# RajeshRk18/exacto

Hardware: AMD Instinct MI355X
Metric: ciphertext muls/sec (bfv_mul_and_relin) (higher is better)
Workload: dtype u64; 1 GPU; bfv_mul_and_relin, BASELINE configs[2]; ring_degree=4096, ct_limbs=3, limb_bits=60, plain_modulus=65537, gadget_base=65536, gadget_digits=12, batch_per_gpu=1024, global_batch=1024, parallelism=batch-shard x1

## Files before the change

### exacto_amd/csrc/arith.hpp

```cpp
#pragma once
#include <hip/hip_runtime.h>
#include <stdint.h>

typedef uint64_t u64;
typedef int64_t i64;
typedef unsigned __int128 u128;
typedef __int128 i128;

#define EXACTO_MAX_L 8
#define EXACTO_MAX_K 10
#define EXACTO_MAX_PRIMES (EXACTO_MAX_L + EXACTO_MAX_K)
#define EXACTO_MAX_G 64

struct __attribute__((aligned(16))) TwPair {
    u64 w;
    u64 ws;
};

struct PrimeConst {
    u64 q, two_q;
    u64 mu64;
    u64 bar_mu;
    int bar_s;
    int pad_;
    u64 n_inv, n_inv_s;
    u64 last_w, last_ws;
    const TwPair* tw_fwd;
    const TwPair* tw_inv;
    u64 qinv_neg;
    u64 n_inv_r, n_inv_rs, last_wr, last_wrs;
};

__device__ __forceinline__ u64 mont_mul_lazy(u64 a, u64 b, u64 q, u64 qinv_neg) {
    const u64 lo = a * b, hi = __umul64hi(a, b);
    const u64 m = lo * qinv_neg;
    return hi + __umul64hi(m, q) + (lo != 0 ? 1 : 0);
}

__device__ __forceinline__ u64 mulhi64(u64 y, u64 s) {
    const uint32_t y0 = (uint32_t)y, y1 = (uint32_t)(y >> 32);
    const uint32_t s0 = (uint32_t)s, s1 = (uint32_t)(s >> 32);
    const u64 u = (u64)y1 * s0 + __umulhi(y0, s0);
    const u128 v = (u128)((u64)y0 * s1) + u;
    return (u64)y1 * s1 + (u64)(v >> 32);
}

// ... 75 lines not shown
```

### exacto_amd/csrc/context.hip

```cpp
#include <algorithm>
#include <cxxabi.h>
#include <dlfcn.h>
#include <chrono>
#include <condition_variable>
#include <cmath>
#include <cstdio>
#include <cstdlib>
#include <cstring>
#include <functional>
#include <map>
#include <memory>
#include <mutex>
#include <set>
#include <string>
#include <thread>
#include <vector>

#include "../../include/exacto_hip.h"
#include "exacto_internal.hpp"

using namespace exacto;

thread_local const void* exacto::g_last_kernel = nullptr;

// ... 648 lines not shown

static int build_tables(exacto_ctx* c) {
    const int NP = (int)c->primes.size();
    std::vector<TwPair> tw((size_t)NP * 2 * c->n);
    std::vector<PrimeConst> pc(NP);
    for (int t = 0; t < NP; ++t)
        pc[t] = make_prime_const(c->primes[t], c->n, c->logn, &tw[(size_t)t * 2 * c->n],
                                 &tw[(size_t)t * 2 * c->n + c->n]);
    HIP_TRY(dev_alloc((void**)&c->d_tw, tw.size() * sizeof(TwPair)));
    if (int e_ = upload(c, c->d_tw, tw.data(), tw.size() * sizeof(TwPair))) return e_;
    for (int t = 0; t < NP; ++t) {
        pc[t].tw_fwd = c->d_tw + (size_t)t * 2 * c->n;
        pc[t].tw_inv = c->d_tw + (size_t)t * 2 * c->n + c->n;
    }
    HIP_TRY(dev_alloc((void**)&c->d_primes, NP * sizeof(PrimeConst)));
    if (int e_ = upload(c, c->d_primes, pc.data(), NP * sizeof(PrimeConst))) return e_;

    CrtTables& C = c->h_crt;
    std::memset(&C, 0, sizeof(C));
    const int L = c->L, K = c->K;
    C.L = L;
    C.K = K;
    C.G = c->G;
    C.gbase = c->gbase;
    C.gshift = (c->gbase & (c->gbase - 1)) == 0 ? bitlen(c->gbase) - 1 : -1;
    C.plain = c->plain;
    const std::vector<u64> qv(c->primes.begin(), c->primes.begin() + L);
    const std::vector<u64> pv(c->primes.begin() + L, c->primes.end());
    for (int i = 0; i < L; ++i)
        for (int k = 0; k < i; ++k) set_shoup(C.gq_w[i][k], C.gq_ws[i][k], invmod_h(qv[k] % qv[i], qv[i]), qv[i]);
    Big Q(1);
// ... 80 lines not shown
                for (int b = 0; b < K; ++b)
                    if (b != a) pm = mulmod_h(pm, pv[b] % qv[i], qv[i]);
                C.fpc_pm[a][i] = pm;
            }
        }
        for (int i = 0; i < L; ++i) {
            const u64 pm = P.mod(qv[i]);
            C.fpc_negP[i] = pm == 0 ? 0 : qv[i] - pm;
        }
        for (int i = 0; i < L; ++i) {
            const u64 q = qv[i];
            u64 qo = 1 % q;
            for (int k = 0; k < L; ++k)
                if (k != i) qo = mulmod_h(qo, qv[k] % q, q);
            set_shoup(C.fpq_pz_w[i], C.fpq_pz_ws[i], mulmod_h(c->plain % q, invmod_h(qo, q), q), q);
            C.fpq_inv0[i] = 1.0 / (double)q;
            C.fpq_inv1[i] = (double)(1ull << 30) / (double)q;
            for (int a = 0; a < K; ++a) {
                const u64 pa = pv[a], qi = invmod_h(q % pa, pa);
                C.fpq_c[i][a] = mulmod_h((pa - qi) % pa, C.fpc_neg[a], pa);
            }
        }
    }
    {
        const u64 mx = *std::max_element(c->primes.begin(), c->primes.end());
        const u64 mn = *std::min_element(c->primes.begin(), c->primes.end());
        C.near = (u128)mx < 2 * (u128)mn;
        C.fast = C.near && mx < (1ull << 60);
        C.special = C.fast && mn > (1ull << 60) - (1ull << 24);
        C.digit_small = c->gbase <= *std::min_element(qv.begin(), qv.end());
    }
    HIP_TRY(dev_alloc((void**)&c->d_scal, EXACTO_MAX_L * sizeof(u64)));
    HIP_TRY(dev_alloc((void**)&c->d_crt, sizeof(CrtTables)));
    if (int e_ = upload(c, c->d_crt, &C, sizeof(CrtTables))) return e_;
    return 0;
}

extern "C" int exacto_ctx_create(exacto_ctx** out, size_t n, const uint64_t* ct_moduli, size_t L,
// ... 341 lines not shown
            CHECK_LAUNCH();
            return 0;
        }
    }
    if (int e = run_ntt(c, nb1, count1, false)) return e;
    return run_ntt(c, nb2, count2, false);
}

static bool tensor_asm(const exacto_ctx* c) {
    bool near60 = c->ntt_asm && c->ntt_asm_inv;
    for (int t = 0; t < c->L + c->K; ++t)
        near60 &= c->primes[t] < (1ull << 60) && c->primes[t] > (1ull << 60) - (1ull << 24);
    return near60;
}

static int run_inv_tensor(exacto_ctx* c, const Operands& o, int cnt, bool p2only = false) {
    const int NP = c->L + c->K;
    bool lazy = true;
    const bool near60 = tensor_asm(c);
    int qbits = 0;
    for (int t = 0; t < NP; ++t) {
        qbits = std::max(qbits, 64 - __builtin_clzll(c->primes[t]));
        lazy &= c->primes[t] < (1ull << 60);
    }
    const double pb = 8.0 * c->n;
    double bytes;
    if (c->tensor_share_d > 0 && c->tensor_share_npairs > 0) {
        const double items = (double)((cnt + c->tensor_share_npairs - 1) / c->tensor_share_npairs);
        const double cts = items * 2.0 * c->tensor_share_d;
        bytes = pb * (c->L * (2.0 * cts + 3.0 * cnt) +
                      c->K * (p2only ? cts + (double)cnt : 2.0 * cts + 3.0 * cnt));
    } else {
        bytes = cnt * (p2only ? pb * (7.0 * c->L + 3.0 * c->K) : pb * 7.0 * NP);
    }
    ProfScope ps(c, PK_TENSOR, (u64)cnt * (p2only ? 3 * c->L + c->K : 3 * NP), bytes);
    launch_inv_tensor(o, c->ws_extP, c->ws_T, cnt, c->logn, c->L, c->K, lazy, c->d_primes, c->stream, near60, p2only,
                      qbits, c->tensor_share_npairs, near60 && c->path != EXACTO_PATH_HPS);
    CHECK_LAUNCH();
    return 0;
}

static NttBatch contiguous(u64* data, long count_items, long poly_per_item, int prime_base, int period,
                           int n) {
    (void)count_items;
    NttBatch nb{};
    nb.src = data;
    nb.src_off = nullptr;
    nb.src_item_stride = poly_per_item * n;
    nb.dst = data;
    nb.dst_item_stride = poly_per_item * n;
    nb.ppi = (int)poly_per_item;
    nb.prime_base = prime_base;
// ... 235 lines not shown
                ProfScope pl(c, PK_HPS_EXT, 4ull * cnt, 8.0 * (1 + K) * n * 4.0 * cnt);
                launch_hps_extend(c->ws_coefQ, c->ws_extP, 4L * cnt, n, c->d_primes, K, c->stream);
            } else {
                ProfScope pl(c, PK_LIFT, 4ull * cnt, 8.0 * (L + K) * n * 4.0 * cnt);
                launch_exact_lift(c->ws_coefQ, c->ws_extP, 4L * cnt, n, c->d_crt, c->d_primes, L, K,
                                  crt_mode(c), c->stream);
            }
            CHECK_LAUNCH();
            NttBatch eb = contiguous(c->ws_extP, cnt, 4L * K, L, K, n);
            eb.lazy_out = c->path != EXACTO_PATH_HPS && tensor_asm(c);
            if (int e = run_ntt(c, eb, (long)cnt * 4 * K, false)) return e;
        } else {
            o.ea_off += s;
            o.eb_off += s;
        }
        if (int e = run_inv_tensor(c, o, cnt, ps.on)) return e;
        if (ps.on) {
            const int ib_cnt = cnt / ps.npairs;
            {
                ProfScope pp(c, PK_PAIRSUM, (u64)ib_cnt * K * ps.d, 8.0 * n * K * ib_cnt * (4.0 * ps.d + 2.0 * ps.d));
                launch_dbfv_pairsum(o, c->ws_extP, ib_cnt, ps.d, ps.npairs, ps.term_start, ps.terms, L, K, n,
                                    c->d_primes, c->stream);
            }
            CHECK_LAUNCH();
            if (int e = run_ntt(c, contiguous(c->ws_extP, (long)ib_cnt * ps.d, 2L * K, L, K, n),
                                (long)ib_cnt * ps.d * 2 * K, true))
                return e;
        }
        u64* R = out + s * out_stride;
        const int ncomp = relin ? 2 : 3;
        u64* D = relin ? c->ws_D : nullptr;
// ... 5 lines not shown
        if (c->path == EXACTO_PATH_HPS) {
            void* d16p = hps_defer ? (c->ks_defer8 ? (void*)((int8_t*)c->ks_defer + s * (long)guse * n)
                                                   : (void*)(c->ks_defer + s * (long)guse * n))
                                   : nullptr;
            launch_hps_scale(c->ws_T, R, out_stride, ncomp, hps_defer ? nullptr : D, d16p,
                             hps_defer && c->ks_defer8, guse, cnt, n, c->d_crt, c->d_primes, K, c->hps_fast,
                             c->stream);
        } else
            launch_exact_scale(c->ws_T, R, out_stride, ncomp, d16 ? nullptr : D,
                               d16 ? (c->ks_defer ? (c->ks_defer8
                                                         ? (int16_t*)((int8_t*)c->ks_defer + s * (long)guse * n)
                                                         : c->ks_defer + s * (long)guse * n)
                                                  : c->ws_D16)
                                   : nullptr,
                               guse, cnt, n, c->d_crt, c->d_primes, L, K, crt_mode(c),
                               c->stream, c->h_crt.gshift, ps.on, c->ks_defer && c->ks_defer8, c->fp_crt, c->fpq_lim);
        CHECK_LAUNCH();
        }
        if (ps.on) {
            const long item0 = s / ps.npairs;
            const double ib = (double)(cnt / ps.npairs);
            ProfScope pq(c, PK_PSUM_SCALE, (u64)(cnt / ps.npairs) * ps.d,
                         ib * 2.0 * n * 8.0 * (ps.d * (double)(K + L) + (double)ps.npairs * L));
            if (!launch_psum_scale(c->ws_T, c->ws_extP, ps.out + item0 * ps.d * 2 * Ln, cnt / ps.npairs, ps.d, ps.npairs,
                                   ps.term_start, ps.terms, n, c->d_crt, c->d_primes, L, c->stream, ps.fpc,
                                   c->fpq_lim))
                return fail(EXACTO_ERR_HIP, "internal: psum scale not available for these limbs");
            CHECK_LAUNCH();
        }
        NttBatch rb{};
        rb.src = R; rb.src_off = nullptr; rb.src_item_stride = out_stride;
// ... 2963 lines not shown
```

### exacto_amd/csrc/exacto_internal.hpp

```cpp
#pragma once
#include "arith.hpp"

namespace exacto {

struct NttBatch {
    const u64* src;
    const u64* src_off;
    long src_item_stride;
    u64* dst;
    long dst_item_stride;
    int ppi;
    int prime_base;
    int period;
    const int16_t* src16;
    long src16_item_stride;
    int lazy_out;
};

enum class MulPath : int { Exact = 0, Hps = 1 };

struct CrtTables {
    int L;
    int K;
    int G;
// ... 10 lines not shown
    u64 halfP_mr[EXACTO_MAX_K];
    u64 ppref_w[EXACTO_MAX_K + 1][EXACTO_MAX_L];
    u64 ppref_ws[EXACTO_MAX_K + 1][EXACTO_MAX_L];
    u64 qinvp_w[EXACTO_MAX_K], qinvp_ws[EXACTO_MAX_K];
    u64 pq_w[EXACTO_MAX_K], pq_ws[EXACTO_MAX_K];
    u64 qpq_w[EXACTO_MAX_L + 1][EXACTO_MAX_K], qpq_ws[EXACTO_MAX_L + 1][EXACTO_MAX_K];
    u64 fpc_pq[EXACTO_MAX_K];
    u64 fpc_qpq[EXACTO_MAX_L][EXACTO_MAX_K];
    u64 fpc_neg[EXACTO_MAX_K];
    double fpc_inv[EXACTO_MAX_K];
    u64 fpc_pm[EXACTO_MAX_K][EXACTO_MAX_L];
    u64 fpc_negP[EXACTO_MAX_L];
    u64 fpq_pz_w[EXACTO_MAX_L], fpq_pz_ws[EXACTO_MAX_L];
    double fpq_inv0[EXACTO_MAX_L], fpq_inv1[EXACTO_MAX_L];
    u64 fpq_c[EXACTO_MAX_L][EXACTO_MAX_K];
    int near;
    int fast;
    int special;
    int digit_small;
    u64 pmod_w[EXACTO_MAX_PRIMES], pmod_ws[EXACTO_MAX_PRIMES];
    u64 Qwords[EXACTO_MAX_L];
    u64 hq[EXACTO_MAX_PRIMES];
    u64 hps_qinv[2];
    u64 hps_p1_inv_p0, hps_p0_inv_p1;
    u64 hps_pc;
    u64 hps_qinv_s[2];
    u64 hps_t_w[2], hps_t_ws[2];
    u64 hps_pq_w[2], hps_pq_ws[2];
    u64 hps_kPq[3];
    u64 hps_P[2], hps_halfP[2];
// ... 54 lines not shown
    const u64* eb;
    const u64* eb_off;
};

bool launch_polymul(const u64* A, const u64* B, u64* out, long rows, int period, int logn, const PrimeConst* primes,
                    hipStream_t s);
void launch_mul_inv(const u64* A, const u64* B, u64* out, long rows, int period, int logn, bool lazy, bool asm_inv,
                    const PrimeConst* primes, hipStream_t s);
struct DropPrimeK {
    u64 w[EXACTO_MAX_L], ws[EXACTO_MAX_L];
};
void launch_drop_prime(const u64* in, u64* out, long rows, int l, bool round, const DropPrimeK& C, int logn, bool lazy,
                       bool asm_rounds, const PrimeConst* primes, hipStream_t s);
void launch_inv_tensor(const Operands& op, const u64* extP, u64* T, int items, int logn, int L, int K, bool lazy,
                       const PrimeConst* primes, hipStream_t s, bool asm_inv = false, bool p2only = false,
                       int qbits = 64, int share_np = 0, bool lazy_out = false);
void launch_phase(const u64* ct, int polys, long ct_stride, const u64* sk, u64* out, int items, int n, int L,
                  const PrimeConst* primes, hipStream_t s);
void launch_decrypt_round(const u64* X, u64* out, int items, int n, int L, const CrtTables* ct,
                          const PrimeConst* primes, u64 plain, hipStream_t s);
int noise_chunks(int n);
void launch_noise(const u64* X, const u64* expected, u64* plain_out, u64* part, u64* out, long items, int group,
                  int n, int L, const CrtTables* ct, const PrimeConst* primes, const u64* delta, u64 plain,
                  bool round, hipStream_t s);
void launch_dbfv_recompose(const u64* digits, u64* out, int items, int n, int d, u64 base, u64 plain, u64 t,
                           bool scalar, hipStream_t s);
void launch_exact_lift(const u64* coefQ, u64* extP, long rows, int n, const CrtTables* ct,
                       const PrimeConst* primes, int L, int K, int mode, hipStream_t s);
void launch_hps_extend(const u64* coefQ, u64* extP, long rows, int n, const PrimeConst* primes,
                       int K, hipStream_t s);
bool exact_scale_sp_ok(int L, int K, int mode);
void launch_exact_scale(const u64* T, u64* R, long r_stride, int ncomp_r, u64* D, int16_t* D16, int guse,
                        int items, int n, const CrtTables* ct, const PrimeConst* primes, int L,
                        int K, int mode, hipStream_t s, int gshift = -1, bool c2only = false,
                        bool digits8 = false, bool fpc = false, double fpq_lim = 0.0);
void launch_hps_scale(const u64* T, u64* R, long r_stride, int ncomp_r, u64* D, void* D16, bool d8, int guse,
                      int items, int n, const CrtTables* ct, const PrimeConst* primes, int K, bool fast,
                      hipStream_t s);
void launch_decompose(const u64* C2, long c2_stride, u64* D, int guse, int items, int n,
                      const CrtTables* ct, const PrimeConst* primes, int L, hipStream_t s, int16_t* D16 = nullptr);
void launch_rows(u64* dst, long dst_stride, const u64* src, long src_stride, long len, long rows, hipStream_t s);
void launch_copy_u64(u64* dst, const u64* src, long words, hipStream_t s);
void launch_xcd_probe(const u64* src, u64* dst, long words, uint32_t* xcc, int blocks, hipStream_t s);
void launch_fill_u32(uint32_t* dst, uint32_t v, long words, hipStream_t s);
void debug_watch_set(const void* lo, const void* hi, uint32_t* hit, hipStream_t s = nullptr);
void launch_relin_mac(const u64* base, long base_stride, const u64* D, const u64* rlk, const u64* rlk_s,
                      int guse, u64* out, long out_stride, int items, int n, int L, const PrimeConst* primes,
                      hipStream_t s);

enum class PwOp : int { Add = 0, Sub = 1, Neg = 2, Mul = 3, ScalarMul = 4, Copy = 5 };
// ... 74 lines not shown
```

### exacto_amd/csrc/kernels.hip

```cpp
#include "exacto_internal.hpp"
#include "crt_dev.hpp"

#include <cstdlib>

namespace exacto {

static constexpr int TPB = 256;

static inline int blocks_per_row(int n) { return (n + TPB - 1) / TPB; }

#define ROW_SETUP(n)                                                   \
    const int nblk = (n + TPB - 1) / TPB;                              \
    const int nsh = __builtin_ctz((unsigned)nblk);                     \
    const long row = (long)(blockIdx.x >> nsh);                        \
    const int j = (int)(blockIdx.x & (unsigned)(nblk - 1)) * TPB + threadIdx.x; \
    if (j >= (n)) return;




template <bool SP>
__device__ __forceinline__ u64 reduce_any(u64 x, const PrimeConst& P) {
    return SP ? reduce_near60(x, P.q) : reduce64(x, P.q, P.mu64);
}
// ... 413 lines not shown
        y0[a] = (uint32_t)y[a] & M30;
        y1[a] = (uint32_t)(y[a] >> 30);
    }
    const uint32_t alpha = (uint32_t)__double2int_rn(f);
#pragma unroll
    for (int i = 0; i < L; ++i) {
        const u64 q = primes[i].q;
        Dot30 A{0, 0, 0};
        dot30_mac(A, alpha, 0, C->fpc_negP[i]);
#pragma unroll
        for (int a = 0; a < K; ++a) dot30_mac(A, y0[a], y1[a], C->fpc_pm[a][i]);
        res[i] = dot30_fold(A, q);
    }
}

template <int LT, bool TA>
__device__ __forceinline__ void fpc_y_garner(const u64* __restrict__ Tin, int n, u64 (&y)[LT + 1],
                                             const CrtTables* __restrict__ C, const PrimeConst* __restrict__ primes) {
    constexpr int L = LT, K = LT + 1;
    u64 u[EXACTO_MAX_L], v[EXACTO_MAX_L];
#pragma unroll
    for (int i = 0; i < L; ++i) u[i] = shoup_mul(Tin[(long)i * n], C->pmod_w[i], C->pmod_ws[i], primes[i].q);
    garner_q_fast<LT>(v, u, L, C, primes);
    const bool negs = mr_greater<EXACTO_MAX_L>(v, C->halfQ_mr, L);
    uint32_t v0[L], v1[L];
#pragma unroll
    for (int k = 0; k < L; ++k) {
        v0[k] = (uint32_t)v[k] & M30;
        v1[k] = (uint32_t)(v[k] >> 30);
    }
#pragma unroll
    for (int a = 0; a < K; ++a) {
        Dot30 A{(TA ? 0ull : y[a]) + (negs ? C->fpc_neg[a] : 0ull), 0, 0};
        if constexpr (TA) {
            const u64 ta = Tin[(long)(L + a) * n];
            dot30_mac(A, (uint32_t)ta & M30, (uint32_t)(ta >> 30), C->fpc_pq[a]);
        }
#pragma unroll
        for (int k = 0; k < L; ++k) dot30_mac(A, v0[k], v1[k], C->fpc_qpq[k][a]);
        y[a] = dot30_fold(A, primes[L + a].q);
    }
}

template <int LT, bool TA>
__device__ __forceinline__ void fpq_y(const u64* __restrict__ Tin, int n, u64 (&y)[LT + 1], const CrtTables* __restrict__ C,
                                      const PrimeConst* __restrict__ primes, double lim) {
    constexpr int L = LT, K = LT + 1;
    uint32_t z0[L], z1[L];
    double f = 0.0;
#pragma unroll
    for (int i = 0; i < L; ++i) {
        const u64 z = shoup_mul_red(Tin[(long)i * n], C->fpq_pz_w[i], C->fpq_pz_ws[i], primes[i].q);
        z0[i] = (uint32_t)z & M30;
        z1[i] = (uint32_t)(z >> 30);
        f = fma((double)z0[i], C->fpq_inv0[i], f);
        f = fma((double)z1[i], C->fpq_inv1[i], f);
    }
    const double b = __builtin_rint(f);
    if (__builtin_fabs(f - b) <= lim) {
        const uint32_t beta = (uint32_t)b;
#pragma unroll
        for (int a = 0; a < K; ++a) {
            Dot30 A{TA ? 0ull : y[a], 0, 0};
            dot30_mac(A, beta, 0, C->fpc_neg[a]);
            if constexpr (TA) {
                const u64 ta = Tin[(long)(L + a) * n];
                dot30_mac(A, (uint32_t)ta & M30, (uint32_t)(ta >> 30), C->fpc_pq[a]);
            }
#pragma unroll
            for (int i = 0; i < L; ++i) dot30_mac(A, z0[i], z1[i], C->fpq_c[i][a]);
            y[a] = dot30_fold(A, primes[L + a].q);
        }
    } else {
        fpc_y_garner<LT, TA>(Tin, n, y, C, primes);
    }
}

template <int LT>
__device__ __forceinline__ void fpq_acc(const u64* __restrict__ Tin, int n, u64 (&Z)[LT], uint32_t& bs, u64 (&carry)[LT + 1],
                                        const CrtTables* __restrict__ C, const PrimeConst* __restrict__ primes,
                                        double lim) {
    constexpr int L = LT;
    u64 z[L];
    double f = 0.0;
#pragma unroll
    for (int i = 0; i < L; ++i) {
        z[i] = shoup_mul_red(Tin[(long)i * n], C->fpq_pz_w[i], C->fpq_pz_ws[i], primes[i].q);
        f = fma((double)((uint32_t)z[i] & M30), C->fpq_inv0[i], f);
        f = fma((double)(uint32_t)(z[i] >> 30), C->fpq_inv1[i], f);
// ... 29 lines not shown
        Z[i] = 0;
    }
#pragma unroll
    for (int a = 0; a < K; ++a) {
        const u64 pa = primes[L + a].q;
        Dot30 A{carry[a], 0, 0};
        dot30_mac(A, bs, 0, C->fpc_neg[a]);
        dot30_mac(A, ks, 0, pa - C->fpc_neg[a]);
#pragma unroll
        for (int i = 0; i < L; ++i) dot30_mac(A, z0[i], z1[i], C->fpq_c[i][a]);
        carry[a] = dot30_fold(A, pa);
    }
    bs = 0;
}

template <int LT, int DIG, bool FPC, bool FPQ = false>
__global__ void __launch_bounds__(TPB)
exact_scale_sp_kernel(const u64* __restrict__ T, u64* __restrict__ R, long r_stride, int ncomp_r,
                      u64* __restrict__ D, int16_t* __restrict__ D16, int guse, int n,
                      const CrtTables* __restrict__ C, const PrimeConst* __restrict__ primes, int c2only,
                      double fpq_lim = 0.0) {
    ROW_SETUP(n)
    constexpr int L = LT, K = LT + 1, NP = L + K;
    const long item = c2only ? row : row / 3;
    const int comp = c2only ? 2 : (int)(row - item * 3);
    const u64* Tin = T + (item * 3 + comp) * NP * n + j;
    u64 res[EXACTO_MAX_L];
    if constexpr (FPQ) {
        static_assert(FPC, "FPQ feeds the float lift from P");
        u64 y[K];
        fpq_y<LT, true>(Tin, n, y, C, primes, fpq_lim);
        fpc_lift<LT>(y, res, C, primes);
    } else {
    u64 u[EXACTO_MAX_L], v[EXACTO_MAX_L];
#pragma unroll
    for (int i = 0; i < L; ++i) u[i] = shoup_mul(Tin[(long)i * n], C->pmod_w[i], C->pmod_ws[i], primes[i].q);
    garner_q_fast<LT>(v, u, L, C, primes);
    const bool negs = mr_greater<EXACTO_MAX_L>(v, C->halfQ_mr, L);
    uint32_t v0[L], v1[L];
#pragma unroll
    for (int k = 0; k < L; ++k) {
        v0[k] = (uint32_t)v[k] & M30;
        v1[k] = (uint32_t)(v[k] >> 30);
    }
    if constexpr (FPC) {
        u64 y[K];
// ... 177 lines not shown
    switch (L) {
        case 1: PSUM_(1); break;
        case 2: PSUM_(2); break;
        case 3: PSUM_(3); break;
        case 4: PSUM_(4); break;
        case 5: PSUM_(5); break;
        case 6: PSUM_(6); break;
        default: return false;
    }
#undef PSUM_
    return true;
}

bool exact_scale_sp_ok(int L, int K, int mode) { return mode == 3 && K == L + 1 && L >= 1 && L <= 6 && use_dot30(); }

void launch_exact_scale(const u64* T, u64* R, long r_stride, int ncomp_r, u64* D, int16_t* D16, int guse,
                        int items, int n, const CrtTables* ct, const PrimeConst* primes, int L,
                        int K, int mode, hipStream_t s, int gshift, bool c2only, bool digits8, bool fpc,
                        double fpq_lim) {
    const long blocks = (long)items * (c2only ? 1 : 3) * blocks_per_row(n);
    if (blocks == 0) return;
    if (mode == 3 && K == L + 1 && L >= 1 && L <= 6 && use_dot30()) {
        const int dig = (D16 == nullptr && D == nullptr) || guse <= 0 ? 0
                        : (D16 != nullptr && gshift > 0 && 32 % gshift == 0) ? (digits8 && gshift <= 8 ? 3 : 1) : 2;
#define SCALE30_(LT, DG)                                                                                        \
    do {                                                                                                        \
        if (fpc && fpq_lim > 0.0)                                                                               \
            EXACTO_LAUNCH((exact_scale_sp_kernel<LT, DG, true, true>), dim3(blocks), dim3(TPB), 0, s, T, R,     \
                          r_stride, ncomp_r, D, D16, guse, n, ct, primes, c2only ? 1 : 0, fpq_lim);             \
        else if (fpc) EXACTO_LAUNCH((exact_scale_sp_kernel<LT, DG, true>), dim3(blocks), dim3(TPB), 0, s, T, R, \
                               r_stride, ncomp_r, D, D16, guse, n, ct, primes, c2only ? 1 : 0, 0.0);            \
        else EXACTO_LAUNCH((exact_scale_sp_kernel<LT, DG, false>), dim3(blocks), dim3(TPB), 0, s, T, R,         \
                           r_stride, ncomp_r, D, D16, guse, n, ct, primes, c2only ? 1 : 0, 0.0);                \
    } while (0)
#define SCALE30(LT)                         \
    do {                                    \
        if (dig == 1) SCALE30_(LT, 1);      \
        else if (dig == 3) SCALE30_(LT, 3); \
        else if (dig == 2) SCALE30_(LT, 2); \
        else SCALE30_(LT, 0);               \
    } while (0)
        switch (L) {
// ... 630 lines not shown
```

### exacto_amd/csrc/ntt.hip

```cpp
#include "exacto_internal.hpp"
#include "ks32_dev.hpp"
#include "bufmem.hpp"
#include "crt_dev.hpp"

namespace exacto {

#ifndef EXACTO_TW_AS
#define EXACTO_TW_AS 1
#endif
#if EXACTO_TW_AS == 0
typedef const TwPair* TwTab;
#else
typedef const TwPair __attribute__((address_space(EXACTO_TW_AS)))* TwTab;
#endif

__device__ __forceinline__ TwTab tw_table(const TwPair* p) { return (TwTab)p; }

__device__ __forceinline__ TwPair ld_tw(TwTab tab, int i) {
    TwPair t;
    t.w = tab[i].w;
    t.ws = tab[i].ws;
    return t;
}

// ... 191 lines not shown
#pragma unroll
    for (int k = 0; k < 16; ++k) {
        u64 v = x[k];
        if (LAZY) {
            v = v >= q8 ? v - q8 : v;
            v = v >= 4 * q ? v - 4 * q : v;
        }
        v = v >= q2 ? v - q2 : v;
        x[k] = v >= q ? v - q : v;
    }
    store_evals<N>(dst, x, tid);
}


#include "ntt_asm.inc"

template <int LO>
__device__ __forceinline__ int lds_base_bytes(int tid) {
    return swz(((tid >> LO) << (LO + 4)) | (tid & ((1 << LO) - 1))) << 3;
}

template <int LO>
__device__ __forceinline__ void lds_store_x(u64* lds, const u64 (&x)[16], int tid) {
    char* lb = reinterpret_cast<char*>(lds);
    const int b = lds_base_bytes<LO>(tid);
#pragma unroll
    for (int k = 0; k < 16; ++k) *reinterpret_cast<u64*>(lb + (b ^ (swz(k << LO) << 3))) = x[k];
}

template <int LO>
// ... 489 lines not shown
        const long ib = g / LQ;
        const int t = (int)(g - ib * LQ), c = w / np, pi = w - c * np;
        prod = ib * np + pi;
        rem = 3 * t + c;
    } else {
        const long bb = b - nQ;
        const long p = remap ? xcd_group_remap(bb, total - nQ, np) : bb;
        const long g = p / np;
        const int pi = (int)(p - g * np);
        const long ib = g / K;
        prod = ib * np + pi;
        rem = 3 * L + (int)(g - ib * K);
    }
}

template <int LOGN, bool LAZY, bool ASM = false, int PROBE = 0, bool GEN = false, int QB = 60, bool LZO = false>
__global__ void __launch_bounds__((1 << LOGN) / 16 < 64 ? 64 : (1 << LOGN) / 16)
__attribute__((amdgpu_waves_per_eu(3)))
ntt_inv_tensor_kernel(Operands op, const u64* __restrict__ extP, u64* __restrict__ Tout, int L, int K,
                      const PrimeConst* __restrict__ primes, int remap, int p2only = 0, int share_np = 0) {
    constexpr int N = 1 << LOGN;
    constexpr int T = N / 16;
    __shared__ u64 lds[N];
    const int tid = T < 64 ? vtid() : (int)threadIdx.x;
    if (tid >= T) return;
    if constexpr (PROBE == 3) probe_stagger<3>(768, EXACTO_PROBE_SLEEPS_TENSOR);
    const int NP = L + K;
    const int per = p2only ? 3 * L + K : 3 * NP;
    long item;
    int rem;
    tensor_block(blockIdx.x, gridDim.x, per, L, K, p2only, share_np, remap, item, rem);
// ... 56 lines not shown
        const u64 q = P.q, q2 = P.two_q;
        if constexpr (ASM) {
            mul16_near60(x, x, y, dq);
#pragma unroll
            for (int k = 0; k < 16; ++k) x[k] += z[k];
        } else {
#pragma unroll
            for (int k = 0; k < 16; ++k) {
                const u64 v = z[k] + mulr(x[k], y[k]);
                x[k] = GEN ? v : LAZY ? (v >= q2 ? v - q2 : v) : (v >= q ? v - q : v);
            }
        }
    }
    if constexpr (PROBE == 2) {
    } else if constexpr (ASM || GEN) {
        const AsmK AK = GEN ? make_asmk_inv_mont(P) : make_asmk_inv(P);
        inv_rounds_asm<LOGN, 0, GEN, QB, LZO && ASM && !GEN>(x, lds, tid, tw_table(P.tw_inv), AK);
    } else {
        inv_rounds<LOGN, 0, LAZY>(x, lds, tid, tw_table(P.tw_inv), P);
    }
    if constexpr (PROBE == 1) {
        if (remap != -7) return;
    }
    u64* dst = Tout + ((item * 3 + c) * NP + t) * N;
    store_evals<N>(dst, x, tid);
}

template <int LOGN, bool LZO = false>
__global__ void __launch_bounds__((1 << LOGN) / 16) __attribute__((amdgpu_waves_per_eu(4)))
ntt_inv_tensor_pin_kernel(Operands op, const u64* __restrict__ extP, u64* __restrict__ Tout, int L, int K,
                          const PrimeConst* __restrict__ primes, int remap, int p2only, int share_np) {
    static_assert(LOGN == 12 || LOGN == 13, "pinned rounds exist for n = 4096 and 8192");
    constexpr int N = 1 << LOGN;
    __shared__ u64 lds[N];
    const int tid = threadIdx.x;
    const int NP = L + K;
    const int per = p2only ? 3 * L + K : 3 * NP;
    long item;
    int rem;
    tensor_block(blockIdx.x, gridDim.x, per, L, K, p2only, share_np, remap, item, rem);
    int t, c;
    tensor_unit(rem, L, p2only, t, c);
    const PrimeConst& P = primes[t];
// ... 30 lines not shown
    } else {
        const PolyRd sa0(A0, N * 8), sa1(A1, N * 8), sb0(B0, N * 8), sb1(B1, N * 8);
#define PIN_T2(k0, k1)                                                   \
        {                                                          \
            u64 r0_, r1_, s0_, s1_;                                \
            MulNear60PinAsm<2>::run(r0_, r1_, LDE(sa0, k0), LDE(sb1, k0), LDE(sa0, k1), LDE(sb1, k1), dq, e16); \
            MulNear60PinAsm<2>::run(s0_, s1_, LDE(sa1, k0), LDE(sb0, k0), LDE(sa1, k1), LDE(sb0, k1), dq, e16); \
            PIN_SET(k0, r0_ + s0_) PIN_SET(k1, r1_ + s1_)          \
        }
        PIN_T2(0, 1) PIN_T2(2, 3) PIN_T2(4, 5) PIN_T2(6, 7)
        __builtin_amdgcn_sched_barrier(0);
        PIN_T2(8, 9) PIN_T2(10, 11) PIN_T2(12, 13) PIN_T2(14, 15)
#undef PIN_T2
    }
#undef LDE
    if constexpr (LZO) {
        PIN_INV_ROUNDS(LOGN, lds, tid, tw_table(P.tw_inv), make_asmk_inv(P), _LZ)
    } else {
        PIN_INV_ROUNDS(LOGN, lds, tid, tw_table(P.tw_inv), make_asmk_inv(P), )
    }
    u64* dst = Tout + ((item * 3 + c) * NP + t) * N;
    {
        const PolyWr rd(dst, N * 8);
#define PIN_OUT(k) rd.st64(PIN_GET(k), tid * 8, (k) * (N / 16) * 8);
        PIN_X16(PIN_OUT)
#undef PIN_OUT
    }
}


template <int LOGN, bool LAZY, bool ASM = false>
// ... 343 lines not shown

static bool ntt_gen_on() {
    static const int on = env_switch("EXACTO_NTT_GEN", 1);
    return on != 0;
}

template <int LOGN>
static bool gen_small(int qbits) {
    static const int on = env_switch("EXACTO_NTT_GENQ", 1);
    return on && gen_qb<LOGN>() < 60 && qbits <= gen_qb<LOGN>();
}

template <int LOGN>
static void launch_it(const Operands& op, const u64* extP, u64* T, long blocks, int L, int K, bool lazy,
                      const PrimeConst* primes, hipStream_t s, bool asm_inv = false, int p2only = 0, int qbits = 64,
                      int np = 0, bool lzo = false) {
    constexpr int threads = (1 << LOGN) / 16;
    static const int remap = [] { const char* e = std::getenv("EXACTO_XCD_REMAP"); return (e && e[0] == '0') ? 0 : 1; }();
    if constexpr (LOGN == 12 || LOGN == 13) {
        if (asm_inv && tensor_pin_at(LOGN)) {
            const long b2 = p2only ? blocks / (3 * (L + K)) * (3 * L + K) : blocks;
            if (lzo)
                EXACTO_LAUNCH((ntt_inv_tensor_pin_kernel<LOGN, true>), dim3(b2), dim3(threads), 0, s, op, extP, T,
                                   L, K, primes, remap, p2only, np);
            else
                EXACTO_LAUNCH((ntt_inv_tensor_pin_kernel<LOGN>), dim3(b2), dim3(threads), 0, s, op, extP, T, L,
                                   K, primes, remap, p2only, np);
            return;
        }
        if (asm_inv) {
            const long b2 = p2only ? blocks / (3 * (L + K)) * (3 * L + K) : blocks;
            if (lzo)
                EXACTO_LAUNCH((ntt_inv_tensor_kernel<LOGN, true, true, 0, false, 60, true>), dim3(b2),
                                   dim3(threads), 0, s, op, extP, T, L, K, primes, remap, p2only, np);
            else
                EXACTO_LAUNCH((ntt_inv_tensor_kernel<LOGN, true, true>), dim3(b2), dim3(threads), 0, s, op, extP,
                                   T, L, K, primes, remap, p2only, np);
            return;
        }
    }
    if constexpr (LOGN == 10 || LOGN == 12 || LOGN == 13) {
        if (lazy && !p2only && ntt_gen_on()) {
            if (gen_small<LOGN>(qbits))
                EXACTO_LAUNCH((ntt_inv_tensor_kernel<LOGN, true, false, 0, true, gen_qb<LOGN>()>), dim3(blocks),
                                   dim3(threads), 0, s, op, extP, T, L, K, primes, remap, 0, np);
            else
                EXACTO_LAUNCH((ntt_inv_tensor_kernel<LOGN, true, false, 0, true>), dim3(blocks), dim3(threads), 0,
                                   s, op, extP, T, L, K, primes, remap, 0, np);
            return;
        }
    }
    if (lazy)
        EXACTO_LAUNCH((ntt_inv_tensor_kernel<LOGN, true>), dim3(blocks), dim3(threads), 0, s, op, extP, T, L, K,
                           primes, remap);
    else
        EXACTO_LAUNCH((ntt_inv_tensor_kernel<LOGN, false>), dim3(blocks), dim3(threads), 0, s, op, extP, T, L,
                           K, primes, remap);
}

void launch_inv_tensor(const Operands& op, const u64* extP, u64* T, int items, int logn, int L, int K, bool lazy,
                       const PrimeConst* primes, hipStream_t s, bool asm_inv, bool p2only, int qbits, int share_np,
                       bool lazy_out) {
    if (share_np < 8 || items % share_np != 0) share_np = 0;
    const long blocks = (long)items * 3 * (L + K);
    if (blocks == 0) return;
    if (p2only) {
        if (logn == 12) launch_it<12>(op, extP, T, blocks, L, K, lazy, primes, s, true, 1, 64, share_np, lazy_out);
        else if (logn == 13) launch_it<13>(op, extP, T, blocks, L, K, lazy, primes, s, true, 1, 64, share_np, lazy_out);
        return;
    }
    switch (logn) {
        case 4: launch_it<4>(op, extP, T, blocks, L, K, lazy, primes, s); break;
        case 5: launch_it<5>(op, extP, T, blocks, L, K, lazy, primes, s); break;
        case 6: launch_it<6>(op, extP, T, blocks, L, K, lazy, primes, s); break;
        case 7: launch_it<7>(op, extP, T, blocks, L, K, lazy, primes, s); break;
        case 8: launch_it<8>(op, extP, T, blocks, L, K, lazy, primes, s); break;
        case 9: launch_it<9>(op, extP, T, blocks, L, K, lazy, primes, s); break;
        case 10: launch_it<10>(op, extP, T, blocks, L, K, lazy, primes, s, false, 0, qbits, share_np); break;
        case 11: launch_it<11>(op, extP, T, blocks, L, K, lazy, primes, s); break;
        case 12: launch_it<12>(op, extP, T, blocks, L, K, lazy, primes, s, asm_inv, 0, qbits, share_np, lazy_out); break;
        case 13: launch_it<13>(op, extP, T, blocks, L, K, lazy, primes, s, asm_inv, 0, qbits, share_np, lazy_out); break;
        case 14: launch_it<14>(op, extP, T, blocks, L, K, lazy, primes, s); break;
        default: break;
    }
}

bool launch_ntt_fwd2(const NttBatch& nb1, int count1, const NttBatch& nb2, int count2, int logn,
                     const PrimeConst* primes, hipStream_t s) {
    if (count1 <= 0 || count2 <= 0 || (logn != 12 && logn != 13)) return false;
    const dim3 grid((unsigned)(count1 + count2));
    if (logn == 12) EXACTO_LAUNCH((ntt_fwd_pin_kernel<12>), grid, dim3(256), 0, s, nb1, primes, nb2, count1);
    else EXACTO_LAUNCH((ntt_fwd_pin_kernel<13>), grid, dim3(512), 0, s, nb1, primes, nb2, count1);
    return true;
}

// ... 58 lines not shown
```

Measured before the change: 469,700 bfv_mul_and_relin/s.

## Fold CRT scale constants into inverse-NTT final multiply for tensor

Precomputes per-prime folded constants (n^-1 and last twiddle pre-multiplied by the exact-scale CRT factors) and uses them in the inverse tensor NTT when logn=12 on the asm lazy-out path. The exact-scale kernel then skips its per-coefficient Shoup multiplies on the Q limbs and the dot30 MAC on the P limbs, using the tensor outputs directly. This removes a multiply stage per limb from the scaling step but couples the two kernels through a shared fold flag and adds template variants.

```diff
diff --git a/exacto_amd/csrc/arith.hpp b/exacto_amd/csrc/arith.hpp
--- a/exacto_amd/csrc/arith.hpp
+++ b/exacto_amd/csrc/arith.hpp
@@ -29,7 +29,12 @@
     const TwPair* tw_inv;
     u64 qinv_neg;
     u64 n_inv_r, n_inv_rs, last_wr, last_wrs;
+    u64 fold_n, fold_ns, fold_w, fold_ws;
 };
+
+#ifndef EXACTO_CRT_FOLD
+#define EXACTO_CRT_FOLD 1
+#endif
 
 __device__ __forceinline__ u64 mont_mul_lazy(u64 a, u64 b, u64 q, u64 qinv_neg) {
     const u64 lo = a * b, hi = __umul64hi(a, b);
diff --git a/exacto_amd/csrc/context.hip b/exacto_amd/csrc/context.hip
--- a/exacto_amd/csrc/context.hip
+++ b/exacto_amd/csrc/context.hip
@@ -686,7 +686,6 @@
         pc[t].tw_inv = c->d_tw + (size_t)t * 2 * c->n + c->n;
     }
     HIP_TRY(dev_alloc((void**)&c->d_primes, NP * sizeof(PrimeConst)));
-    if (int e_ = upload(c, c->d_primes, pc.data(), NP * sizeof(PrimeConst))) return e_;
 
     CrtTables& C = c->h_crt;
     std::memset(&C, 0, sizeof(C));
@@ -797,6 +796,7 @@
             for (int k = 0; k < L; ++k)
                 if (k != i) qo = mulmod_h(qo, qv[k] % q, q);
             set_shoup(C.fpq_pz_w[i], C.fpq_pz_ws[i], mulmod_h(c->plain % q, invmod_h(qo, q), q), q);
+            set_shoup(C.fpq_qo_w[i], C.fpq_qo_ws[i], qo, q);
             C.fpq_inv0[i] = 1.0 / (double)q;
             C.fpq_inv1[i] = (double)(1ull << 30) / (double)q;
             for (int a = 0; a < K; ++a) {
@@ -804,7 +804,14 @@
                 C.fpq_c[i][a] = mulmod_h((pa - qi) % pa, C.fpc_neg[a], pa);
             }
         }
-    }
+        auto fold = [&](PrimeConst& P, u64 f) {
+            set_shoup(P.fold_n, P.fold_ns, mulmod_h(P.n_inv, f, P.q), P.q);
+            set_shoup(P.fold_w, P.fold_ws, mulmod_h(P.last_w, f, P.q), P.q);
+        };
+        for (int i = 0; i < L; ++i) fold(pc[i], C.fpq_pz_w[i]);
+        for (int a = 0; a < K; ++a) fold(pc[L + a], C.fpc_pq[a]);
+    }
+    if (int e_ = upload(c, c->d_primes, pc.data(), NP * sizeof(PrimeConst))) return e_;
     {
         const u64 mx = *std::max_element(c->primes.begin(), c->primes.end());
         const u64 mn = *std::min_element(c->primes.begin(), c->primes.end());
@@ -1176,7 +1183,13 @@
     return near60;
 }
 
-static int run_inv_tensor(exacto_ctx* c, const Operands& o, int cnt, bool p2only = false) {
+static int crt_mode(const exacto_ctx* c);
+static bool scale_fold(const exacto_ctx* c) {
+    return c->path != EXACTO_PATH_HPS && crt_fold_tensor_ok(c->logn, tensor_asm(c), true) &&
+           exact_scale_fold_ok(c->L, c->K, crt_mode(c), c->fp_crt, c->fpq_lim);
+}
+
+static int run_inv_tensor(exacto_ctx* c, const Operands& o, int cnt, bool p2only = false, bool fold = false) {
     const int NP = c->L + c->K;
     bool lazy = true;
     const bool near60 = tensor_asm(c);
@@ -1197,7 +1210,7 @@
     }
     ProfScope ps(c, PK_TENSOR, (u64)cnt * (p2only ? 3 * c->L + c->K : 3 * NP), bytes);
     launch_inv_tensor(o, c->ws_extP, c->ws_T, cnt, c->logn, c->L, c->K, lazy, c->d_primes, c->stream, near60, p2only,
-                      qbits, c->tensor_share_npairs, near60 && c->path != EXACTO_PATH_HPS);
+                      qbits, c->tensor_share_npairs, near60 && c->path != EXACTO_PATH_HPS, fold);
     CHECK_LAUNCH();
     return 0;
 }
@@ -1463,7 +1476,8 @@
             o.ea_off += s;
             o.eb_off += s;
         }
-        if (int e = run_inv_tensor(c, o, cnt, ps.on)) return e;
+        const bool tfold = !ps.on && scale_fold(c);
+        if (int e = run_inv_tensor(c, o, cnt, ps.on, tfold)) return e;
         if (ps.on) {
             const int ib_cnt = cnt / ps.npairs;
             {
@@ -1499,7 +1513,8 @@
                                                   : c->ws_D16)
                                    : nullptr,
                                guse, cnt, n, c->d_crt, c->d_primes, L, K, crt_mode(c),
-                               c->stream, c->h_crt.gshift, ps.on, c->ks_defer && c->ks_defer8, c->fp_crt, c->fpq_lim);
+                               c->stream, c->h_crt.gshift, ps.on, c->ks_defer && c->ks_defer8, c->fp_crt, c->fpq_lim,
+                               tfold);
         CHECK_LAUNCH();
         }
         if (ps.on) {
diff --git a/exacto_amd/csrc/exacto_internal.hpp b/exacto_amd/csrc/exacto_internal.hpp
--- a/exacto_amd/csrc/exacto_internal.hpp
+++ b/exacto_amd/csrc/exacto_internal.hpp
@@ -48,6 +48,7 @@
     u64 fpq_pz_w[EXACTO_MAX_L], fpq_pz_ws[EXACTO_MAX_L];
     double fpq_inv0[EXACTO_MAX_L], fpq_inv1[EXACTO_MAX_L];
     u64 fpq_c[EXACTO_MAX_L][EXACTO_MAX_K];
+    u64 fpq_qo_w[EXACTO_MAX_L], fpq_qo_ws[EXACTO_MAX_L];
     int near;
     int fast;
     int special;
@@ -132,7 +133,8 @@
                        bool asm_rounds, const PrimeConst* primes, hipStream_t s);
 void launch_inv_tensor(const Operands& op, const u64* extP, u64* T, int items, int logn, int L, int K, bool lazy,
                        const PrimeConst* primes, hipStream_t s, bool asm_inv = false, bool p2only = false,
-                       int qbits = 64, int share_np = 0, bool lazy_out = false);
+                       int qbits = 64, int share_np = 0, bool lazy_out = false, bool fold = false);
+bool crt_fold_tensor_ok(int logn, bool asm_inv, bool lazy_out);
 void launch_phase(const u64* ct, int polys, long ct_stride, const u64* sk, u64* out, int items, int n, int L,
                   const PrimeConst* primes, hipStream_t s);
 void launch_decrypt_round(const u64* X, u64* out, int items, int n, int L, const CrtTables* ct,
@@ -151,7 +153,8 @@
 void launch_exact_scale(const u64* T, u64* R, long r_stride, int ncomp_r, u64* D, int16_t* D16, int guse,
                         int items, int n, const CrtTables* ct, const PrimeConst* primes, int L,
                         int K, int mode, hipStream_t s, int gshift = -1, bool c2only = false,
-                        bool digits8 = false, bool fpc = false, double fpq_lim = 0.0);
+                        bool digits8 = false, bool fpc = false, double fpq_lim = 0.0, bool fold = false);
+bool exact_scale_fold_ok(int L, int K, int mode, bool fpc, double fpq_lim);
 void launch_hps_scale(const u64* T, u64* R, long r_stride, int ncomp_r, u64* D, void* D16, bool d8, int guse,
                       int items, int n, const CrtTables* ct, const PrimeConst* primes, int K, bool fast,
                       hipStream_t s);
diff --git a/exacto_amd/csrc/kernels.hip b/exacto_amd/csrc/kernels.hip
--- a/exacto_amd/csrc/kernels.hip
+++ b/exacto_amd/csrc/kernels.hip
@@ -451,13 +451,16 @@
     }
 }
 
-template <int LT, bool TA>
+template <int LT, bool TA, bool FOLD = false>
 __device__ __forceinline__ void fpc_y_garner(const u64* __restrict__ Tin, int n, u64 (&y)[LT + 1],
                                              const CrtTables* __restrict__ C, const PrimeConst* __restrict__ primes) {
     constexpr int L = LT, K = LT + 1;
+    static_assert(!FOLD || TA, "the folded tensor feeds the scale alone");
     u64 u[EXACTO_MAX_L], v[EXACTO_MAX_L];
 #pragma unroll
-    for (int i = 0; i < L; ++i) u[i] = shoup_mul(Tin[(long)i * n], C->pmod_w[i], C->pmod_ws[i], primes[i].q);
+    for (int i = 0; i < L; ++i)
+        u[i] = FOLD ? shoup_mul(Tin[(long)i * n], C->fpq_qo_w[i], C->fpq_qo_ws[i], primes[i].q)
+                    : shoup_mul(Tin[(long)i * n], C->pmod_w[i], C->pmod_ws[i], primes[i].q);
     garner_q_fast<LT>(v, u, L, C, primes);
     const bool negs = mr_greater<EXACTO_MAX_L>(v, C->halfQ_mr, L);
     uint32_t v0[L], v1[L];
@@ -469,7 +472,9 @@
 #pragma unroll
     for (int a = 0; a < K; ++a) {
         Dot30 A{(TA ? 0ull : y[a]) + (negs ? C->fpc_neg[a] : 0ull), 0, 0};
-        if constexpr (TA) {
+        if constexpr (TA && FOLD) {
+            A.a0 += Tin[(long)(L + a) * n];
+        } else if constexpr (TA) {
             const u64 ta = Tin[(long)(L + a) * n];
             dot30_mac(A, (uint32_t)ta & M30, (uint32_t)(ta >> 30), C->fpc_pq[a]);
         }
@@ -479,15 +484,17 @@
     }
 }
 
-template <int LT, bool TA>
+template <int LT, bool TA, bool FOLD = false>
 __device__ __forceinline__ void fpq_y(const u64* __restrict__ Tin, int n, u64 (&y)[LT + 1], const CrtTables* __restrict__ C,
                                       const PrimeConst* __restrict__ primes, double lim) {
     constexpr int L = LT, K = LT + 1;
+    static_assert(!FOLD || (TA && LT <= 5), "folded form: the scale's own tensor, L <= 5 (dot budget)");
     uint32_t z0[L], z1[L];
     double f = 0.0;
 #pragma unroll
     for (int i = 0; i < L; ++i) {
-        const u64 z = shoup_mul_red(Tin[(long)i * n], C->fpq_pz_w[i], C->fpq_pz_ws[i], primes[i].q);
+        const u64 z = FOLD ? Tin[(long)i * n]
+                           : shoup_mul_red(Tin[(long)i * n], C->fpq_pz_w[i], C->fpq_pz_ws[i], primes[i].q);
         z0[i] = (uint32_t)z & M30;
         z1[i] = (uint32_t)(z >> 30);
         f = fma((double)z0[i], C->fpq_inv0[i], f);
@@ -498,9 +505,9 @@
         const uint32_t beta = (uint32_t)b;
 #pragma unroll
         for (int a = 0; a < K; ++a) {
-            Dot30 A{TA ? 0ull : y[a], 0, 0};
+            Dot30 A{TA ? (FOLD ? Tin[(long)(L + a) * n] : 0ull) : y[a], 0, 0};
             dot30_mac(A, beta, 0, C->fpc_neg[a]);
-            if constexpr (TA) {
+            if constexpr (TA && !FOLD) {
                 const u64 ta = Tin[(long)(L + a) * n];
                 dot30_mac(A, (uint32_t)ta & M30, (uint32_t)(ta >> 30), C->fpc_pq[a]);
             }
@@ -509,7 +516,7 @@
             y[a] = dot30_fold(A, primes[L + a].q);
         }
     } else {
-        fpc_y_garner<LT, TA>(Tin, n, y, C, primes);
+        fpc_y_garner<LT, TA, FOLD>(Tin, n, y, C, primes);
     }
 }
 
@@ -569,7 +576,7 @@
     bs = 0;
 }
 
-template <int LT, int DIG, bool FPC, bool FPQ = false>
+template <int LT, int DIG, bool FPC, bool FPQ = false, bool FOLD = false>
 __global__ void __launch_bounds__(TPB)
 exact_scale_sp_kernel(const u64* __restrict__ T, u64* __restrict__ R, long r_stride, int ncomp_r,
                       u64* __restrict__ D, int16_t* __restrict__ D16, int guse, int n,
@@ -584,7 +591,7 @@
     if constexpr (FPQ) {
         static_assert(FPC, "FPQ feeds the float lift from P");
         u64 y[K];
-        fpq_y<LT, true>(Tin, n, y, C, primes, fpq_lim);
+        fpq_y<LT, true, FOLD>(Tin, n, y, C, primes, fpq_lim);
         fpc_lift<LT>(y, res, C, primes);
     } else {
     u64 u[EXACTO_MAX_L], v[EXACTO_MAX_L];
@@ -792,18 +799,27 @@
 
 bool exact_scale_sp_ok(int L, int K, int mode) { return mode == 3 && K == L + 1 && L >= 1 && L <= 6 && use_dot30(); }
 
+bool exact_scale_fold_ok(int L, int K, int mode, bool fpc, double fpq_lim) {
+    return EXACTO_CRT_FOLD && exact_scale_sp_ok(L, K, mode) && L <= 5 && fpc && fpq_lim > 0.0;
+}
+
 void launch_exact_scale(const u64* T, u64* R, long r_stride, int ncomp_r, u64* D, int16_t* D16, int guse,
                         int items, int n, const CrtTables* ct, const PrimeConst* primes, int L,
                         int K, int mode, hipStream_t s, int gshift, bool c2only, bool digits8, bool fpc,
-                        double fpq_lim) {
+                        double fpq_lim, bool fold) {
     const long blocks = (long)items * (c2only ? 1 : 3) * blocks_per_row(n);
     if (blocks == 0) return;
     if (mode == 3 && K == L + 1 && L >= 1 && L <= 6 && use_dot30()) {
         const int dig = (D16 == nullptr && D == nullptr) || guse <= 0 ? 0
                         : (D16 != nullptr && gshift > 0 && 32 % gshift == 0) ? (digits8 && gshift <= 8 ? 3 : 1) : 2;
+        const bool folded = fold && exact_scale_fold_ok(L, K, mode, fpc, fpq_lim);
 #define SCALE30_(LT, DG)                                                                                        \
     do {                                                                                                        \
-        if (fpc && fpq_lim > 0.0)                                                                               \
+        if (folded)                                                                                             \
+            EXACTO_LAUNCH((exact_scale_sp_kernel<LT, DG, true, true, (EXACTO_CRT_FOLD != 0 && LT <= 5)>),       \
+                          dim3(blocks), dim3(TPB), 0, s, T, R, r_stride, ncomp_r, D, D16, guse, n, ct, primes,  \
+                          c2only ? 1 : 0, fpq_lim);                                                             \
+        else if (fpc && fpq_lim > 0.0)                                                                          \
             EXACTO_LAUNCH((exact_scale_sp_kernel<LT, DG, true, true>), dim3(blocks), dim3(TPB), 0, s, T, R,     \
                           r_stride, ncomp_r, D, D16, guse, n, ct, primes, c2only ? 1 : 0, fpq_lim);             \
         else if (fpc) EXACTO_LAUNCH((exact_scale_sp_kernel<LT, DG, true>), dim3(blocks), dim3(TPB), 0, s, T, R, \
diff --git a/exacto_amd/csrc/ntt.hip b/exacto_amd/csrc/ntt.hip
--- a/exacto_amd/csrc/ntt.hip
+++ b/exacto_amd/csrc/ntt.hip
@@ -229,6 +229,15 @@
 
 
 #include "ntt_asm.inc"
+
+__device__ __forceinline__ AsmK make_asmk_inv_fold(const PrimeConst& P) {
+    AsmK K = make_asmk(P.q);
+    K.nil = (uint32_t)P.fold_n; K.nih = (uint32_t)(P.fold_n >> 32);
+    K.nsl = (uint32_t)P.fold_ns; K.nsh = (uint32_t)(P.fold_ns >> 32);
+    K.lwl = (uint32_t)P.fold_w; K.lwh = (uint32_t)(P.fold_w >> 32);
+    K.lsl = (uint32_t)P.fold_ws; K.lsh = (uint32_t)(P.fold_ws >> 32);
+    return K;
+}
 
 template <int LO>
 __device__ __forceinline__ int lds_base_bytes(int tid) {
@@ -748,7 +757,8 @@
     }
 }
 
-template <int LOGN, bool LAZY, bool ASM = false, int PROBE = 0, bool GEN = false, int QB = 60, bool LZO = false>
+template <int LOGN, bool LAZY, bool ASM = false, int PROBE = 0, bool GEN = false, int QB = 60, bool LZO = false,
+          bool FOLD = false>
 __global__ void __launch_bounds__((1 << LOGN) / 16 < 64 ? 64 : (1 << LOGN) / 16)
 __attribute__((amdgpu_waves_per_eu(3)))
 ntt_inv_tensor_kernel(Operands op, const u64* __restrict__ extP, u64* __restrict__ Tout, int L, int K,
@@ -835,7 +845,8 @@
     }
     if constexpr (PROBE == 2) {
     } else if constexpr (ASM || GEN) {
-        const AsmK AK = GEN ? make_asmk_inv_mont(P) : make_asmk_inv(P);
+        static_assert(!FOLD || (ASM && !GEN), "the folded constants exist for the special-prime rounds");
+        const AsmK AK = GEN ? make_asmk_inv_mont(P) : FOLD ? make_asmk_inv_fold(P) : make_asmk_inv(P);
         inv_rounds_asm<LOGN, 0, GEN, QB, LZO && ASM && !GEN>(x, lds, tid, tw_table(P.tw_inv), AK);
     } else {
         inv_rounds<LOGN, 0, LAZY>(x, lds, tid, tw_table(P.tw_inv), P);
@@ -847,7 +858,7 @@
     store_evals<N>(dst, x, tid);
 }
 
-template <int LOGN, bool LZO = false>
+template <int LOGN, bool LZO = false, bool FOLD = false>
 __global__ void __launch_bounds__((1 << LOGN) / 16) __attribute__((amdgpu_waves_per_eu(4)))
 ntt_inv_tensor_pin_kernel(Operands op, const u64* __restrict__ extP, u64* __restrict__ Tout, int L, int K,
                           const PrimeConst* __restrict__ primes, int remap, int p2only, int share_np) {
@@ -908,7 +919,9 @@
 #undef PIN_T2
     }
 #undef LDE
-    if constexpr (LZO) {
+    if constexpr (LZO && FOLD) {
+        PIN_INV_ROUNDS(LOGN, lds, tid, tw_table(P.tw_inv), make_asmk_inv_fold(P), _LZ)
+    } else if constexpr (LZO) {
         PIN_INV_ROUNDS(LOGN, lds, tid, tw_table(P.tw_inv), make_asmk_inv(P), _LZ)
     } else {
         PIN_INV_ROUNDS(LOGN, lds, tid, tw_table(P.tw_inv), make_asmk_inv(P), )
@@ -1282,12 +1295,21 @@
 template <int LOGN>
 static void launch_it(const Operands& op, const u64* extP, u64* T, long blocks, int L, int K, bool lazy,
                       const PrimeConst* primes, hipStream_t s, bool asm_inv = false, int p2only = 0, int qbits = 64,
-                      int np = 0, bool lzo = false) {
+                      int np = 0, bool lzo = false, bool fold = false) {
     constexpr int threads = (1 << LOGN) / 16;
     static const int remap = [] { const char* e = std::getenv("EXACTO_XCD_REMAP"); return (e && e[0] == '0') ? 0 : 1; }();
     if constexpr (LOGN == 12 || LOGN == 13) {
         if (asm_inv && tensor_pin_at(LOGN)) {
             const long b2 = p2only ? blocks / (3 * (L + K)) * (3 * L + K) : blocks;
+#if EXACTO_CRT_FOLD
+            if constexpr (LOGN == 12) {
+                if (lzo && fold) {
+                    EXACTO_LAUNCH((ntt_inv_tensor_pin_kernel<LOGN, true, true>), dim3(b2), dim3(threads), 0, s, op,
+                                       extP, T, L, K, primes, remap, p2only, np);
+                    return;
+                }
+            }
+#endif
             if (lzo)
                 EXACTO_LAUNCH((ntt_inv_tensor_pin_kernel<LOGN, true>), dim3(b2), dim3(threads), 0, s, op, extP, T,
                                    L, K, primes, remap, p2only, np);
@@ -1298,6 +1320,15 @@
         }
         if (asm_inv) {
             const long b2 = p2only ? blocks / (3 * (L + K)) * (3 * L + K) : blocks;
+#if EXACTO_CRT_FOLD
+            if constexpr (LOGN == 12) {
+                if (lzo && fold) {
+                    EXACTO_LAUNCH((ntt_inv_tensor_kernel<LOGN, true, true, 0, false, 60, true, true>), dim3(b2),
+                                       dim3(threads), 0, s, op, extP, T, L, K, primes, remap, p2only, np);
+                    return;
+                }
+            }
+#endif
             if (lzo)
                 EXACTO_LAUNCH((ntt_inv_tensor_kernel<LOGN, true, true, 0, false, 60, true>), dim3(b2),
                                    dim3(threads), 0, s, op, extP, T, L, K, primes, remap, p2only, np);
@@ -1326,9 +1357,13 @@
                            K, primes, remap);
 }
 
+bool crt_fold_tensor_ok(int logn, bool asm_inv, bool lazy_out) {
+    return EXACTO_CRT_FOLD && EXACTO_MUL_ASM && logn == 12 && asm_inv && lazy_out;
+}
+
 void launch_inv_tensor(const Operands& op, const u64* extP, u64* T, int items, int logn, int L, int K, bool lazy,
                        const PrimeConst* primes, hipStream_t s, bool asm_inv, bool p2only, int qbits, int share_np,
-                       bool lazy_out) {
+                       bool lazy_out, bool fold) {
     if (share_np < 8 || items % share_np != 0) share_np = 0;
     const long blocks = (long)items * 3 * (L + K);
     if (blocks == 0) return;
@@ -1346,7 +1381,10 @@
         case 9: launch_it<9>(op, extP, T, blocks, L, K, lazy, primes, s); break;
         case 10: launch_it<10>(op, extP, T, blocks, L, K, lazy, primes, s, false, 0, qbits, share_np); break;
         case 11: launch_it<11>(op, extP, T, blocks, L, K, lazy, primes, s); break;
-        case 12: launch_it<12>(op, extP, T, blocks, L, K, lazy, primes, s, asm_inv, 0, qbits, share_np, lazy_out); break;
+        case 12:
+            launch_it<12>(op, extP, T, blocks, L, K, lazy, primes, s, asm_inv, 0, qbits, share_np, lazy_out,
+                          fold && crt_fold_tensor_ok(logn, asm_inv, lazy_out));
+            break;
         case 13: launch_it<13>(op, extP, T, blocks, L, K, lazy, primes, s, asm_inv, 0, qbits, share_np, lazy_out); break;
         case 14: launch_it<14>(op, extP, T, blocks, L, K, lazy, primes, s); break;
         default: break;
```

After: 478,000 bfv_mul_and_relin/s (median of 6 runs). +1.8%, better.
